# Nightmare-n/GD-MAE

Hardware: AMD Instinct MI355X
Metric: MAE pre-train frames/sec (Waymo-shape, 180k pts, 75% mask) (higher is better)
Workload: dtype bf16

## Files before the change

gd-mae_amd/csrc/vfe_fused.hip:

```cpp
#include "common.h"
#include "gemm.h"

int gd_bn_fold_from_partials(hipStream_t st, const float* part, int nblk, int C, double count, const float* gamma,
                             const float* beta, double eps, double momentum, float* running_mean, float* running_var,
                             long long* num_batches, double* stats, float* ab, float* mv);
int gd_partials_to_f64(hipStream_t st, const float* part, int nblk, int C2, double* out);
extern "C" int gdmae_bn_bwd_coeffs(const double* st, int n_st, const double* stats, const float* ab, const float* gamma, int C,
                                   double count, const double* tot, float* dgamma, float* dbeta, int accumulate, float* c01,
                                   void* stream);

namespace {

typedef float f32x16 __attribute__((ext_vector_type(16)));

constexpr int VF_C = 64;
constexpr int VF_WAVES = 4;
constexpr int VF_MAX_GRID = 1024;

struct VfeGeom {
  float lo[3], vs[3];
  int out_f16 = 0;
};

enum { VF_STATS = 0, VF_APPLY = 1, VF_BSTATS = 2, VF_DW = 3 };

__device__ inline unsigned short vf_f2bf(float f) { return gd_to_bf16(f); }

template <int F>
struct VfA {
  float r[F + 1];
  int pil;
};
struct VfB {
  long long c1, c2, c3;
  float m[3];
};
template <int F>
__device__ __forceinline__ void vf_load_a(const float* __restrict__ pts, const int* __restrict__ inv, long long i, long long N, VfA<F>& A) {
  const long long ic = i < N ? i : N - 1;
  const float* r = pts + ic * (F + 1);
#pragma unroll
  for (int k = 0; k < F + 1; ++k) A.r[k] = r[k];
  A.pil = inv[ic];
}
template <int F>
__device__ __forceinline__ void vf_load_b(const long long* __restrict__ coords, const float* __restrict__ mean, int cpp, long long i,
                                          long long N, int pil, VfB& B) {
  const long long ic = i < N ? i : N - 1;
  const long long* c = coords + 4 * (cpp ? (long long)pil : ic);
  const float* m = mean + (long long)pil * F;
  B.c1 = c[1]; B.c2 = c[2]; B.c3 = c[3];
  B.m[0] = m[0]; B.m[1] = m[1]; B.m[2] = m[2];
}
template <int F>
__device__ __forceinline__ void vf_features(const VfA<F>& A, const VfB& B, bool live, const VfeGeom& G, float (&f)[F + 6]) {
  const float x = A.r[1], y = A.r[2], z = A.r[3];
  f[0] = __fsub_rn(x, __fadd_rn(__fmul_rn(__fadd_rn((float)B.c3, 0.5f), G.vs[0]), G.lo[0]));
  f[1] = __fsub_rn(y, __fadd_rn(__fmul_rn(__fadd_rn((float)B.c2, 0.5f), G.vs[1]), G.lo[1]));
  f[2] = __fsub_rn(z, __fadd_rn(__fmul_rn(__fadd_rn((float)B.c1, 0.5f), G.vs[2]), G.lo[2]));
#pragma unroll
  for (int k = 0; k < F; ++k) f[3 + k] = A.r[1 + k];
  f[3 + F] = __fsub_rn(x, B.m[0]);
  f[4 + F] = __fsub_rn(y, B.m[1]);
  f[5 + F] = __fsub_rn(z, B.m[2]);
#pragma unroll
  for (int k = 0; k < F + 6; ++k) f[k] = live ? f[k] : 0.f;
}
template <bool BF>
struct VfG {
  unsigned u[BF ? 16 : 1];
  float2 v[BF ? 1 : 16];
};
template <bool BF>
__device__ __forceinline__ void vf_load_g(const void* __restrict__ g, long long base, long long N, int n, int half, VfG<BF>& Gr) {
#pragma unroll
  for (int r = 0; r < 16; ++r) {
    const long long row = base + 8 * (r / 4) + 4 * half + (r % 4);
    const long long rc = row < N ? row : N - 1;
    if (BF) Gr.u[r] = ((const unsigned*)g)[rc * (VF_C / 2) + n];
    else Gr.v[r] = ((const float2*)g)[rc * (VF_C / 2) + n];
  }
}

template <int F, int MODE, bool BF>
__global__ __launch_bounds__(VF_WAVES * 64) void k_vfe1(const float* __restrict__ pts, const long long* __restrict__ coords,
                                                        const int* __restrict__ inv, const float* __restrict__ mean,
                                                        int cpp, long long N, VfeGeom G, const float* __restrict__ W,
                                                        const float* __restrict__ ab, const float* __restrict__ c01,
                                                        const void* __restrict__ g, void* __restrict__ out,
                                                        float* __restrict__ part) {
  constexpr int D = F + 6;
  constexpr int KS = (D + 1) / 2;
  constexpr int DP = 2 * KS;
  const int lane = threadIdx.x & 63, wave = threadIdx.x >> 6;
  const int n = lane & 31, half = lane >> 5;
  __shared__ float sh[VF_WAVES * (MODE == VF_DW ? VF_C * D : 4 * VF_C)];
  __shared__ float shf[MODE == VF_DW ? VF_WAVES * 32 * DP : 1];

  float wb[2][KS];
#pragma unroll
  for (int blk = 0; blk < 2; ++blk)
#pragma unroll
    for (int s = 0; s < KS; ++s) {
      const int d = 2 * s + half;
      wb[blk][s] = d < D ? W[(2 * n + blk) * D + d] : 0.f;
    }
  float ca[2] = {0.f, 0.f}, cb[2] = {0.f, 0.f}, c0[2] = {0.f, 0.f}, c1[2] = {0.f, 0.f};
  if (MODE != VF_STATS) {
#pragma unroll
    for (int blk = 0; blk < 2; ++blk) {
      ca[blk] = ab[2 * n + blk];
      cb[blk] = ab[VF_C + 2 * n + blk];
      if (MODE == VF_DW) {
        c0[blk] = c01[2 * n + blk];
        c1[blk] = c01[VF_C + 2 * n + blk];
      }
    }
  }
  float s1[2] = {0.f, 0.f}, s2[2] = {0.f, 0.f};
  f32x16 accw[2];
#pragma unroll
  for (int r = 0; r < 16; ++r) accw[0][r] = accw[1][r] = 0.f;

  const long long ntiles = (N + 31) / 32;
  const long long tstride = (long long)gridDim.x * VF_WAVES;
  constexpr bool HAS_G = MODE == VF_BSTATS || MODE == VF_DW;
  constexpr bool PIPE = !HAS_G;
  VfA<F> A1, A2, A3;
  VfB B1, B2;
  VfG<BF> G1;
  if (PIPE) {
    const long long t = (long long)blockIdx.x * VF_WAVES + wave;
    vf_load_a<F>(pts, inv, t * 32 + n, N, A1);
    vf_load_a<F>(pts, inv, (t + tstride) * 32 + n, N, A2);
    vf_load_b<F>(coords, mean, cpp, t * 32 + n, N, A1.pil, B1);
  }
  for (long long t0 = (long long)blockIdx.x * VF_WAVES; t0 < ntiles; t0 += tstride) {
    const long long base = (t0 + wave) * 32;
    if (PIPE) {
      vf_load_a<F>(pts, inv, base + 2 * tstride * 32 + n, N, A3);
      vf_load_b<F>(coords, mean, cpp, base + tstride * 32 + n, N, A2.pil, B2);
      __builtin_amdgcn_sched_barrier(0);
    } else {
      vf_load_g<BF>(g, base, N, n, half, G1);
      vf_load_a<F>(pts, inv, base + n, N, A1);
      vf_load_b<F>(coords, mean, cpp, base + n, N, A1.pil, B1);
    }
    float g0[16], g1[16];
    if (HAS_G) {
#pragma unroll
      for (int r = 0; r < 16; ++r) {
        const long long row = base + 8 * (r / 4) + 4 * half + (r % 4);
        if (BF) {
          g0[r] = row < N ? __uint_as_float(G1.u[r] << 16) : 0.f;
          g1[r] = row < N ? __uint_as_float(G1.u[r] & 0xFFFF0000u) : 0.f;
        } else {
          g0[r] = row < N ? G1.v[r].x : 0.f;
          g1[r] = row < N ? G1.v[r].y : 0.f;
        }
      }
    }
    float f[D];
    vf_features<F>(A1, B1, base + n < N, G, f);
    f32x16 h[2];
#pragma unroll
    for (int r = 0; r < 16; ++r) h[0][r] = h[1][r] = 0.f;
#pragma unroll
    for (int s = 0; s < KS; ++s) {
      const float f0 = f[2 * s], f1 = (2 * s + 1 < D) ? f[2 * s + 1] : 0.f;
      const float a = half ? f1 : f0;
      h[0] = __builtin_amdgcn_mfma_f32_32x32x2f32(a, wb[0][s], h[0], 0, 0, 0);
      h[1] = __builtin_amdgcn_mfma_f32_32x32x2f32(a, wb[1][s], h[1], 0, 0, 0);
    }
    if (MODE == VF_STATS) {
#pragma unroll
      for (int r = 0; r < 16; ++r)
#pragma unroll
        for (int blk = 0; blk < 2; ++blk) {
          const float v = h[blk][r];
          s1[blk] += v;
          s2[blk] = fmaf(v, v, s2[blk]);
        }
    } else if (MODE == VF_APPLY) {
#pragma unroll
      for (int k = 0; k < F + 1; ++k) asm volatile("" : "+v"(A3.r[k]));
      asm volatile("" : "+v"(A3.pil));
      asm volatile("" : "+v"(B2.c1), "+v"(B2.c2), "+v"(B2.c3), "+v"(B2.m[0]), "+v"(B2.m[1]), "+v"(B2.m[2]));
#pragma unroll
      for (int r = 0; r < 16; ++r) {
        const long long row = base + 8 * (r / 4) + 4 * half + (r % 4);
        if (row < N) {
          const float y0 = fmaxf(fmaf(ca[0], h[0][r], cb[0]), 0.f), y1 = fmaxf(fmaf(ca[1], h[1][r], cb[1]), 0.f);
          if (BF) ((unsigned*)out)[row * (VF_C / 2) + n] = G.out_f16 ? gd_pack_f16(y0, y1) : ((unsigned)vf_f2bf(y0) | ((unsigned)vf_f2bf(y1) << 16));
          else ((float2*)out)[row * (VF_C / 2) + n] = make_float2(y0, y1);
        }
      }
    } else {
      if (MODE == VF_DW) {
        if (half == 0) {
#pragma unroll
          for (int d = 0; d < DP; ++d) shf[(wave * 32 + n) * DP + d] = d < D ? f[d] : 0.f;
        }
        __builtin_amdgcn_fence(__ATOMIC_RELEASE, "wavefront");
        __builtin_amdgcn_wave_barrier();
        __builtin_amdgcn_fence(__ATOMIC_ACQUIRE, "wavefront");
      }
#pragma unroll
      for (int r = 0; r < 16; ++r) {
        const int pr = 8 * (r / 4) + 4 * half + (r % 4);
        const float dh0 = fmaf(ca[0], h[0][r], cb[0]) > 0.f ? g0[r] : 0.f;
        const float dh1 = fmaf(ca[1], h[1][r], cb[1]) > 0.f ? g1[r] : 0.f;
        if (MODE == VF_BSTATS) {
          s1[0] += dh0;
          s1[1] += dh1;
          s2[0] = fmaf(dh0, h[0][r], s2[0]);
          s2[1] = fmaf(dh1, h[1][r], s2[1]);
        } else {
          const float dx0 = fmaf(c1[0], h[0][r], fmaf(ca[0], dh0, c0[0]));
          const float dx1 = fmaf(c1[1], h[1][r], fmaf(ca[1], dh1, c0[1]));
          const float bv = n < DP ? shf[(wave * 32 + pr) * DP + n] : 0.f;
          accw[0] = __builtin_amdgcn_mfma_f32_32x32x2f32(dx0, bv, accw[0], 0, 0, 0);
          accw[1] = __builtin_amdgcn_mfma_f32_32x32x2f32(dx1, bv, accw[1], 0, 0, 0);
        }
      }
      if (MODE == VF_DW) {
        __builtin_amdgcn_fence(__ATOMIC_RELEASE, "wavefront");
        __builtin_amdgcn_wave_barrier();
      }
    }
    if (PIPE) {
      A1 = A2;
      A2 = A3;
      B1 = B2;
    }
  }

  if (MODE == VF_STATS || MODE == VF_BSTATS) {
#pragma unroll
    for (int blk = 0; blk < 2; ++blk) {
      s1[blk] += __shfl_xor(s1[blk], 32, 64);
      s2[blk] += __shfl_xor(s2[blk], 32, 64);
    }
    if (half == 0) {
#pragma unroll
      for (int blk = 0; blk < 2; ++blk) {
        sh[wave * 2 * VF_C + 2 * n + blk] = s1[blk];
        sh[wave * 2 * VF_C + VF_C + 2 * n + blk] = s2[blk];
      }
    }
    __syncthreads();
    if (threadIdx.x < 2 * VF_C) {
      float a = 0.f;
#pragma unroll
      for (int w = 0; w < VF_WAVES; ++w) a += sh[w * 2 * VF_C + threadIdx.x];
      part[(long long)blockIdx.x * 2 * VF_C + threadIdx.x] = a;
    }
  } else if (MODE == VF_DW) {
    if (n < D) {
#pragma unroll
      for (int blk = 0; blk < 2; ++blk)
#pragma unroll
        for (int r = 0; r < 16; ++r) {
          const int col = 2 * (8 * (r / 4) + 4 * half + (r % 4)) + blk;
          sh[wave * VF_C * D + col * D + n] = accw[blk][r];
        }
    }
    __syncthreads();
    for (int e = threadIdx.x; e < VF_C * D; e += VF_WAVES * 64) {
      float a = 0.f;
#pragma unroll
      for (int w = 0; w < VF_WAVES; ++w) a += sh[w * VF_C * D + e];
      part[(long long)blockIdx.x * VF_C * D + e] = a;
    }
  }
}

template <typename K>
int vf_resident_blocks(K kernel, int slot) {
  static int cache[32] = {0};
  if (cache[slot] == 0) {
    int per_cu = 0, dev = 0;
    hipDeviceProp_t prop;
    if (hipOccupancyMaxActiveBlocksPerMultiprocessor(&per_cu, kernel, VF_WAVES * 64, 0) != hipSuccess || per_cu < 1) per_cu = 2;
    if (hipGetDevice(&dev) != hipSuccess || hipGetDeviceProperties(&prop, dev) != hipSuccess) prop.multiProcessorCount = 256;
    const long long b = (long long)per_cu * prop.multiProcessorCount;
    cache[slot] = (int)(b > VF_MAX_GRID ? VF_MAX_GRID : b);
  }
  return cache[slot];
}

template <int MODE>
int vf_launch(hipStream_t st, int F, bool bf, const float* pts, const long long* coords, const int* inv, const float* mean,
              int cpp, long long N, const VfeGeom& G, const float* W, const float* ab, const float* c01, const void* g, void* out,
              float* part, int* grid_out = nullptr) {
  const long long tiles = (N + 31) / 32, blocks = (tiles + VF_WAVES - 1) / VF_WAVES;
  const dim3 block(VF_WAVES * 64);
#define VF_GO(FF, BB)                                                                                                   \
  do {                                                                                                                  \
    const int cap = vf_resident_blocks(k_vfe1<FF, MODE, BB>, ((FF - 3) * 4 + MODE) * 2 + (BB ? 1 : 0));                 \
    const dim3 grid((unsigned)(blocks < cap ? blocks : cap));                                                           \
    if (grid_out) *grid_out = (int)grid.x;                                                                              \
    hipLaunchKernelGGL((k_vfe1<FF, MODE, BB>), grid, block, 0, st, pts, coords, inv, mean, cpp, N, G, W, ab, c01, g, out, part); \
  } while (0)
  if (F == 5) { if (bf) VF_GO(5, true); else VF_GO(5, false); }
  else if (F == 4) { if (bf) VF_GO(4, true); else VF_GO(4, false); }
  else if (F == 3) { if (bf) VF_GO(3, true); else VF_GO(3, false); }
  else GD_REQUIRE(false, "vfe point layer: 3, 4 or 5 point features (x, y, z [, intensity [, elongation]])");
#undef VF_GO
  GD_LAUNCH_CHECK();
  return 0;
}

}

__global__ __launch_bounds__(256) void k_pillar_major_rows(const float* __restrict__ pts, int ncols, const int* __restrict__ csr,
                                                           const int* __restrict__ inv, const int* __restrict__ n_dev,
                                                           float* __restrict__ pts_pm, int* __restrict__ rowpil) {
  const long long N = *n_dev;
  for (long long q = blockIdx.x * (long long)blockDim.x + threadIdx.x; q < N; q += (long long)gridDim.x * blockDim.x) {
    const int i = csr[q];
    rowpil[q] = inv[i];
    for (int k = 0; k < ncols; ++k) pts_pm[q * ncols + k] = pts[(long long)i * ncols + k];
  }
}

extern "C" int gdmae_pillar_major_rows(const float* points, int n_cols, const int* pillar_pts, const int* inverse32,
                                       const int* n_dev, long long capacity, float* points_pm, int* row_pillar,
                                       void* stream) {
  if (capacity <= 0) return 0;
  hipLaunchKernelGGL(k_pillar_major_rows, dim3((unsigned)(capacity / 256 + 1 > 8192 ? 8192 : capacity / 256 + 1)), dim3(256), 0, (hipStream_t)stream, points, n_cols,
                     pillar_pts, inverse32, n_dev, points_pm, row_pillar);
  GD_LAUNCH_CHECK();
  return 0;
}

extern "C" size_t gdmae_vfe_point_layer_workspace_bytes(int n_cols) {
  const int D = n_cols - 1 + 6;
  return gd_align((size_t)VF_MAX_GRID * VF_C * (D > 2 ? D : 2) * sizeof(float)) + gd_align(2 * VF_C * sizeof(double)) +
         gd_align(2 * VF_C * sizeof(float));
}

extern "C" int gdmae_vfe_point_layer_fwd(const float* points, const long long* point_coords, const int* inverse32,
                                         const float* pillar_mean, int coords_per_pillar, long long N, int n_cols,
                                         const float* lo, const float* vs,
                                         const float* W, int C, const float* gamma, const float* beta, double eps,
                                         double momentum, float* running_mean, float* running_var, long long* num_batches,
                                         double* stats, float* ab, float* mv, void* out, int out_bf16, void* workspace,
                                         void* stream) {
  GD_REQUIRE(C == VF_C, "vfe point layer: 64 output channels");
  GD_REQUIRE(N > 0, "vfe point layer: no points");
  hipStream_t st = (hipStream_t)stream;
  VfeGeom G;
  for (int i = 0; i < 3; ++i) { G.lo[i] = lo[i]; G.vs[i] = vs[i]; }
  float* part = (float*)workspace;
  const int F = n_cols - 1;
  int grid = 0;
  int rc = vf_launch<VF_STATS>(st, F, false, points, point_coords, inverse32, pillar_mean, coords_per_pillar, N, G, W, nullptr, nullptr, nullptr,
                               nullptr, part, &grid);
  if (rc) return rc;
  rc = gd_bn_fold_from_partials(st, part, grid, C, (double)N, gamma, beta, eps, momentum, running_mean, running_var,
                                num_batches, stats, ab, mv);
  if (rc) return rc;
  G.out_f16 = out_bf16 == 2;
  return vf_launch<VF_APPLY>(st, F, out_bf16 != 0, points, point_coords, inverse32, pillar_mean, coords_per_pillar, N, G, W, ab, nullptr, nullptr,
                             out, nullptr);
}

extern "C" int gdmae_vfe_point_layer_bwd(const float* points, const long long* point_coords, const int* inverse32,
                                         const float* pillar_mean, int coords_per_pillar, long long N, int n_cols,
                                         const float* lo, const float* vs,
                                         const float* W, int C, const float* gamma, const double* stats, const float* ab,
                                         const void* g, int g_bf16, float* dgamma, float* dbeta, float* dW, int accumulate,
                                         void* workspace, void* stream) {
  GD_REQUIRE(C == VF_C, "vfe point layer: 64 output channels");
  GD_REQUIRE(N > 0, "vfe point layer: no points");
  hipStream_t st = (hipStream_t)stream;
  VfeGeom G;
  for (int i = 0; i < 3; ++i) { G.lo[i] = lo[i]; G.vs[i] = vs[i]; }
  const int F = n_cols - 1, D = F + 6;
  char* p = (char*)workspace;
  float* part = (float*)p;
  p += gd_align((size_t)VF_MAX_GRID * VF_C * (D > 2 ? D : 2) * sizeof(float));
  double* sums = (double*)p;
  p += gd_align(2 * VF_C * sizeof(double));
  float* c01 = (float*)p;
  int grid = 0;
  int rc = vf_launch<VF_BSTATS>(st, F, g_bf16 != 0, points, point_coords, inverse32, pillar_mean, coords_per_pillar, N, G, W, ab, nullptr, g,
                                nullptr, part, &grid);
  if (rc) return rc;
  rc = gd_partials_to_f64(st, part, grid, 2 * C, sums);
  if (rc) return rc;
  rc = gdmae_bn_bwd_coeffs(sums, 2, stats, ab, gamma, C, (double)N, nullptr, dgamma, dbeta, accumulate, c01, stream);
  if (rc) return rc;
  rc = vf_launch<VF_DW>(st, F, g_bf16 != 0, points, point_coords, inverse32, pillar_mean, coords_per_pillar, N, G, W, ab, c01, g, nullptr, part, &grid);
  if (rc) return rc;
  return gd_splitk_acc(st, part, grid, (long long)VF_C * D, dW, accumulate);
}
```

Baseline: 1056.

## Fuse VFE point-layer backward into single pass using feature Gram matrix

```diff
diff --git a/gd-mae_amd/csrc/vfe_fused.hip b/gd-mae_amd/csrc/vfe_fused.hip
--- a/gd-mae_amd/csrc/vfe_fused.hip
+++ b/gd-mae_amd/csrc/vfe_fused.hip
@@ -1,28 +1,26 @@
 #include "common.h"
-#include "gemm.h"
 
 int gd_bn_fold_from_partials(hipStream_t st, const float* part, int nblk, int C, double count, const float* gamma,
                              const float* beta, double eps, double momentum, float* running_mean, float* running_var,
                              long long* num_batches, double* stats, float* ab, float* mv);
-int gd_partials_to_f64(hipStream_t st, const float* part, int nblk, int C2, double* out);
-extern "C" int gdmae_bn_bwd_coeffs(const double* st, int n_st, const double* stats, const float* ab, const float* gamma, int C,
-                                   double count, const double* tot, float* dgamma, float* dbeta, int accumulate, float* c01,
-                                   void* stream);
 
 namespace {
 
 typedef float f32x16 __attribute__((ext_vector_type(16)));
+typedef float f32x4 __attribute__((ext_vector_type(4)));
 
 constexpr int VF_C = 64;
 constexpr int VF_WAVES = 4;
 constexpr int VF_MAX_GRID = 1024;
+constexpr int VF_FS = 16;
+constexpr int vf_bwd_part(int D) { return (VF_C + D + 1) * (D + 1); }
 
 struct VfeGeom {
   float lo[3], vs[3];
   int out_f16 = 0;
 };
 
-enum { VF_STATS = 0, VF_APPLY = 1, VF_BSTATS = 2, VF_DW = 3 };
+enum { VF_STATS = 0, VF_APPLY = 1, VF_BWD = 2 };
 
 __device__ inline unsigned short vf_f2bf(float f) { return gd_to_bf16(f); }
 
@@ -86,16 +84,16 @@
 __global__ __launch_bounds__(VF_WAVES * 64) void k_vfe1(const float* __restrict__ pts, const long long* __restrict__ coords,
                                                         const int* __restrict__ inv, const float* __restrict__ mean,
                                                         int cpp, long long N, VfeGeom G, const float* __restrict__ W,
-                                                        const float* __restrict__ ab, const float* __restrict__ c01,
-                                                        const void* __restrict__ g, void* __restrict__ out,
+                                                        const float* __restrict__ ab, const void* __restrict__ g, void* __restrict__ out,
                                                         float* __restrict__ part) {
   constexpr int D = F + 6;
   constexpr int KS = (D + 1) / 2;
-  constexpr int DP = 2 * KS;
   const int lane = threadIdx.x & 63, wave = threadIdx.x >> 6;
   const int n = lane & 31, half = lane >> 5;
-  __shared__ float sh[VF_WAVES * (MODE == VF_DW ? VF_C * D : 4 * VF_C)];
-  __shared__ float shf[MODE == VF_DW ? VF_WAVES * 32 * DP : 1];
+  constexpr int DQ = D + 1, PW = vf_bwd_part(D);
+  static_assert(DQ <= VF_FS, "feature tile row");
+  __shared__ float sh[VF_WAVES * (MODE == VF_BWD ? PW : 4 * VF_C)];
+  __shared__ __attribute__((aligned(16))) float shf[MODE == VF_BWD ? VF_WAVES * 32 * VF_FS : 4];
 
   float wb[2][KS];
 #pragma unroll
@@ -105,26 +103,26 @@
       const int d = 2 * s + half;
       wb[blk][s] = d < D ? W[(2 * n + blk) * D + d] : 0.f;
     }
-  float ca[2] = {0.f, 0.f}, cb[2] = {0.f, 0.f}, c0[2] = {0.f, 0.f}, c1[2] = {0.f, 0.f};
+  float ca[2] = {0.f, 0.f}, cb[2] = {0.f, 0.f};
   if (MODE != VF_STATS) {
 #pragma unroll
     for (int blk = 0; blk < 2; ++blk) {
       ca[blk] = ab[2 * n + blk];
       cb[blk] = ab[VF_C + 2 * n + blk];
-      if (MODE == VF_DW) {
-        c0[blk] = c01[2 * n + blk];
-        c1[blk] = c01[VF_C + 2 * n + blk];
-      }
     }
   }
   float s1[2] = {0.f, 0.f}, s2[2] = {0.f, 0.f};
   f32x16 accw[2];
 #pragma unroll
   for (int r = 0; r < 16; ++r) accw[0][r] = accw[1][r] = 0.f;
+  f32x4 accf = {0.f, 0.f, 0.f, 0.f};
+  float sft[F];
+#pragma unroll
+  for (int k = 0; k < F; ++k) sft[k] = MODE == VF_BWD ? pts[1 + k] : 0.f;
 
   const long long ntiles = (N + 31) / 32;
   const long long tstride = (long long)gridDim.x * VF_WAVES;
-  constexpr bool HAS_G = MODE == VF_BSTATS || MODE == VF_DW;
+  constexpr bool HAS_G = MODE == VF_BWD;
   constexpr bool PIPE = !HAS_G;
   VfA<F> A1, A2, A3;
   VfB B1, B2;
@@ -147,16 +145,18 @@
       vf_load_b<F>(coords, mean, cpp, base + n, N, A1.pil, B1);
     }
     float g0[16], g1[16];
+    const long long left = N - base;
+    const int nrem = left < 0 ? 0 : (left > 32 ? 32 : (int)left);
     if (HAS_G) {
 #pragma unroll
       for (int r = 0; r < 16; ++r) {
-        const long long row = base + 8 * (r / 4) + 4 * half + (r % 4);
+        const bool ok = 8 * (r / 4) + 4 * half + (r % 4) < nrem;
         if (BF) {
-          g0[r] = row < N ? __uint_as_float(G1.u[r] << 16) : 0.f;
-          g1[r] = row < N ? __uint_as_float(G1.u[r] & 0xFFFF0000u) : 0.f;
+          g0[r] = ok ? __uint_as_float(G1.u[r] << 16) : 0.f;
+          g1[r] = ok ? __uint_as_float(G1.u[r] & 0xFFFF0000u) : 0.f;
         } else {
-          g0[r] = row < N ? G1.v[r].x : 0.f;
-          g1[r] = row < N ? G1.v[r].y : 0.f;
+          g0[r] = ok ? G1.v[r].x : 0.f;
+          g1[r] = ok ? G1.v[r].y : 0.f;
         }
       }
     }
@@ -196,37 +196,37 @@
         }
       }
     } else {
-      if (MODE == VF_DW) {
-        if (half == 0) {
-#pragma unroll
-          for (int d = 0; d < DP; ++d) shf[(wave * 32 + n) * DP + d] = d < D ? f[d] : 0.f;
-        }
-        __builtin_amdgcn_fence(__ATOMIC_RELEASE, "wavefront");
-        __builtin_amdgcn_wave_barrier();
-        __builtin_amdgcn_fence(__ATOMIC_ACQUIRE, "wavefront");
-      }
+      if (half == 0) {
+        const bool live = n < nrem;
+        float t[VF_FS];
+#pragma unroll
+        for (int d = 0; d < VF_FS; ++d) t[d] = d < D ? f[d] : (d == D && live ? 1.f : 0.f);
+#pragma unroll
+        for (int k = 0; k < F; ++k) t[3 + k] = live ? __fsub_rn(f[3 + k], sft[k]) : 0.f;
+#pragma unroll
+        for (int q = 0; q < VF_FS / 4; ++q)
+          ((float4*)shf)[(wave * 32 + n) * (VF_FS / 4) + q] = make_float4(t[4 * q], t[4 * q + 1], t[4 * q + 2], t[4 * q + 3]);
+      }
+      __builtin_amdgcn_fence(__ATOMIC_RELEASE, "wavefront");
+      __builtin_amdgcn_wave_barrier();
+      __builtin_amdgcn_fence(__ATOMIC_ACQUIRE, "wavefront");
+      int tb = (wave * 32 + 4 * half) * VF_FS + (n & (VF_FS - 1));
+      asm volatile("" : "+v"(tb));
 #pragma unroll
       for (int r = 0; r < 16; ++r) {
-        const int pr = 8 * (r / 4) + 4 * half + (r % 4);
         const float dh0 = fmaf(ca[0], h[0][r], cb[0]) > 0.f ? g0[r] : 0.f;
         const float dh1 = fmaf(ca[1], h[1][r], cb[1]) > 0.f ? g1[r] : 0.f;
-        if (MODE == VF_BSTATS) {
-          s1[0] += dh0;
-          s1[1] += dh1;
-          s2[0] = fmaf(dh0, h[0][r], s2[0]);
-          s2[1] = fmaf(dh1, h[1][r], s2[1]);
-        } else {
-          const float dx0 = fmaf(c1[0], h[0][r], fmaf(ca[0], dh0, c0[0]));
-          const float dx1 = fmaf(c1[1], h[1][r], fmaf(ca[1], dh1, c0[1]));
-          const float bv = n < DP ? shf[(wave * 32 + pr) * DP + n] : 0.f;
-          accw[0] = __builtin_amdgcn_mfma_f32_32x32x2f32(dx0, bv, accw[0], 0, 0, 0);
-          accw[1] = __builtin_amdgcn_mfma_f32_32x32x2f32(dx1, bv, accw[1], 0, 0, 0);
-        }
-      }
-      if (MODE == VF_DW) {
-        __builtin_amdgcn_fence(__ATOMIC_RELEASE, "wavefront");
-        __builtin_amdgcn_wave_barrier();
-      }
+        const float bv = shf[tb + (8 * (r / 4) + (r % 4)) * VF_FS];
+        accw[0] = __builtin_amdgcn_mfma_f32_32x32x2f32(dh0, bv, accw[0], 0, 0, 0);
+        accw[1] = __builtin_amdgcn_mfma_f32_32x32x2f32(dh1, bv, accw[1], 0, 0, 0);
+      }
+#pragma unroll
+      for (int s = 0; s < 8; ++s) {
+        const float tv = shf[wave * 32 * VF_FS + s * 64 + lane];
+        accf = __builtin_amdgcn_mfma_f32_16x16x4f32(tv, tv, accf, 0, 0, 0);
+      }
+      __builtin_amdgcn_fence(__ATOMIC_RELEASE, "wavefront");
+      __builtin_amdgcn_wave_barrier();
     }
     if (PIPE) {
       A1 = A2;
@@ -235,7 +235,7 @@
     }
   }
 
-  if (MODE == VF_STATS || MODE == VF_BSTATS) {
+  if (MODE == VF_STATS) {
 #pragma unroll
     for (int blk = 0; blk < 2; ++blk) {
       s1[blk] += __shfl_xor(s1[blk], 32, 64);
@@ -255,29 +255,34 @@
       for (int w = 0; w < VF_WAVES; ++w) a += sh[w * 2 * VF_C + threadIdx.x];
       part[(long long)blockIdx.x * 2 * VF_C + threadIdx.x] = a;
     }
-  } else if (MODE == VF_DW) {
-    if (n < D) {
+  } else if (MODE == VF_BWD) {
+    if (n < DQ) {
 #pragma unroll
       for (int blk = 0; blk < 2; ++blk)
 #pragma unroll
         for (int r = 0; r < 16; ++r) {
           const int col = 2 * (8 * (r / 4) + 4 * half + (r % 4)) + blk;
-          sh[wave * VF_C * D + col * D + n] = accw[blk][r];
+          sh[wave * PW + col * DQ + n] = accw[blk][r];
         }
     }
+#pragma unroll
+    for (int r = 0; r < 4; ++r) {
+      const int i = 4 * (lane >> 4) + r, j = lane & 15;
+      if (i < DQ && j < DQ) sh[wave * PW + (VF_C + i) * DQ + j] = accf[r];
+    }
     __syncthreads();
-    for (int e = threadIdx.x; e < VF_C * D; e += VF_WAVES * 64) {
+    for (int e = threadIdx.x; e < PW; e += VF_WAVES * 64) {
       float a = 0.f;
 #pragma unroll
-      for (int w = 0; w < VF_WAVES; ++w) a += sh[w * VF_C * D + e];
-      part[(long long)blockIdx.x * VF_C * D + e] = a;
+      for (int w = 0; w < VF_WAVES; ++w) a += sh[w * PW + e];
+      part[(long long)blockIdx.x * PW + e] = a;
     }
   }
 }
 
 template <typename K>
 int vf_resident_blocks(K kernel, int slot) {
-  static int cache[32] = {0};
+  static int cache[18] = {0};
   if (cache[slot] == 0) {
     int per_cu = 0, dev = 0;
     hipDeviceProp_t prop;
@@ -291,16 +296,16 @@
 
 template <int MODE>
 int vf_launch(hipStream_t st, int F, bool bf, const float* pts, const long long* coords, const int* inv, const float* mean,
-              int cpp, long long N, const VfeGeom& G, const float* W, const float* ab, const float* c01, const void* g, void* out,
+              int cpp, long long N, const VfeGeom& G, const float* W, const float* ab, const void* g, void* out,
               float* part, int* grid_out = nullptr) {
   const long long tiles = (N + 31) / 32, blocks = (tiles + VF_WAVES - 1) / VF_WAVES;
   const dim3 block(VF_WAVES * 64);
 #define VF_GO(FF, BB)                                                                                                   \
   do {                                                                                                                  \
-    const int cap = vf_resident_blocks(k_vfe1<FF, MODE, BB>, ((FF - 3) * 4 + MODE) * 2 + (BB ? 1 : 0));                 \
+    const int cap = vf_resident_blocks(k_vfe1<FF, MODE, BB>, ((FF - 3) * 3 + MODE) * 2 + (BB ? 1 : 0));                 \
     const dim3 grid((unsigned)(blocks < cap ? blocks : cap));                                                           \
     if (grid_out) *grid_out = (int)grid.x;                                                                              \
-    hipLaunchKernelGGL((k_vfe1<FF, MODE, BB>), grid, block, 0, st, pts, coords, inv, mean, cpp, N, G, W, ab, c01, g, out, part); \
+    hipLaunchKernelGGL((k_vfe1<FF, MODE, BB>), grid, block, 0, st, pts, coords, inv, mean, cpp, N, G, W, ab, g, out, part); \
   } while (0)
   if (F == 5) { if (bf) VF_GO(5, true); else VF_GO(5, false); }
   else if (F == 4) { if (bf) VF_GO(4, true); else VF_GO(4, false); }
@@ -311,6 +316,67 @@
   return 0;
 }
 
+constexpr int VF_FIN_CH = 8, VF_FIN_SL = 4, VF_FIN_E = 256;
+__global__ __launch_bounds__(VF_FIN_SL * VF_FIN_E) void k_vfe1_finish(const float* __restrict__ part, int S, int D,
+                                                                      const float* __restrict__ pts, const float* __restrict__ W,
+                                                                      const double* __restrict__ stats, const float* __restrict__ ab,
+                                                                      const float* __restrict__ gamma, double count,
+                                                                      float* __restrict__ dgamma, float* __restrict__ dbeta,
+                                                                      float* __restrict__ dW, int accumulate) {
+  __shared__ double sh[VF_FIN_SL][VF_FIN_E];
+  __shared__ double T[VF_FIN_E];
+  const int DQ = D + 1, PW = (VF_C + DQ) * DQ, E = VF_FIN_CH * DQ + DQ * DQ;
+  const int e = threadIdx.x % VF_FIN_E, sl = threadIdx.x / VF_FIN_E;
+  {
+    const int ec = e < E ? e : E - 1;
+    const float* p = part + (ec < VF_FIN_CH * DQ ? blockIdx.x * VF_FIN_CH * DQ + ec : VF_C * DQ + (ec - VF_FIN_CH * DQ));
+    const int s0 = (S * sl) / VF_FIN_SL, s1 = (S * (sl + 1)) / VF_FIN_SL;
+    double acc = 0.0;
+    for (int b0 = s0; b0 < s1; b0 += 16) {
+      float v[16];
+#pragma unroll
+      for (int u = 0; u < 16; ++u) v[u] = p[(long long)(b0 + u < s1 ? b0 + u : s1 - 1) * PW];
+#pragma unroll
+      for (int u = 0; u < 16; ++u) acc += b0 + u < s1 ? (double)v[u] : 0.0;
+    }
+    sh[sl][e] = acc;
+  }
+  __syncthreads();
+  if (threadIdx.x < VF_FIN_E) {
+    double a = 0.0;
+#pragma unroll
+    for (int k = 0; k < VF_FIN_SL; ++k) a += sh[k][threadIdx.x];
+    T[threadIdx.x] = a;
+  }
+  __syncthreads();
+  if (threadIdx.x >= VF_FIN_CH * D) return;
+  const int cl = threadIdx.x / D, d = threadIdx.x % D, c = blockIdx.x * VF_FIN_CH + cl;
+  const double* Pc = T + cl * DQ;
+  const double* M = T + VF_FIN_CH * DQ;
+  auto shift = [&](int k) { return k >= 3 && k < D - 3 ? (double)pts[k - 2] : 0.0; };
+  const double db = Pc[D];
+  double dhh = 0.0, wff = 0.0;
+  const double sd = shift(d), fsd = M[D * DQ + d] + count * sd;
+  for (int k = 0; k < D; ++k) {
+    const double w = (double)W[c * D + k], sk = shift(k);
+    dhh += w * (Pc[k] + db * sk);
+    wff += w * (M[k * DQ + d] + sk * M[D * DQ + d] + M[D * DQ + k] * sd + count * sk * sd);
+  }
+  const double mean = stats[c], r = stats[VF_C + c], a = (double)ab[c];
+  const double da = dhh - db * mean;
+  const double dv = -0.5 * (da * (double)gamma[c]) * r * r * r;
+  const double dmu = -db * a - 2.0 * mean * dv;
+  const double c0 = dmu / count, c1 = 2.0 * dv / count;
+  const float dw = (float)(a * (Pc[d] + db * sd) + c0 * fsd + c1 * wff);
+  if (accumulate) dW[c * D + d] += dw;
+  else dW[c * D + d] = dw;
+  if (d == 0) {
+    const float dg = (float)(da * r), dbf = (float)db;
+    if (accumulate) { dgamma[c] += dg; dbeta[c] += dbf; }
+    else { dgamma[c] = dg; dbeta[c] = dbf; }
+  }
+}
+
 }
 
 __global__ __launch_bounds__(256) void k_pillar_major_rows(const float* __restrict__ pts, int ncols, const int* __restrict__ csr,
@@ -335,9 +401,8 @@
 }
 
 extern "C" size_t gdmae_vfe_point_layer_workspace_bytes(int n_cols) {
-  const int D = n_cols - 1 + 6;
-  return gd_align((size_t)VF_MAX_GRID * VF_C * (D > 2 ? D : 2) * sizeof(float)) + gd_align(2 * VF_C * sizeof(double)) +
-         gd_align(2 * VF_C * sizeof(float));
+  const int D = n_cols - 1 + 6, pw = vf_bwd_part(D > 0 ? D : 0);
+  return gd_align((size_t)VF_MAX_GRID * (pw > 2 * VF_C ? pw : 2 * VF_C) * sizeof(float));
 }
 
 extern "C" int gdmae_vfe_point_layer_fwd(const float* points, const long long* point_coords, const int* inverse32,
@@ -355,14 +420,14 @@
   float* part = (float*)workspace;
   const int F = n_cols - 1;
   int grid = 0;
-  int rc = vf_launch<VF_STATS>(st, F, false, points, point_coords, inverse32, pillar_mean, coords_per_pillar, N, G, W, nullptr, nullptr, nullptr,
+  int rc = vf_launch<VF_STATS>(st, F, false, points, point_coords, inverse32, pillar_mean, coords_per_pillar, N, G, W, nullptr, nullptr,
                                nullptr, part, &grid);
   if (rc) return rc;
   rc = gd_bn_fold_from_partials(st, part, grid, C, (double)N, gamma, beta, eps, momentum, running_mean, running_var,
                                 num_batches, stats, ab, mv);
   if (rc) return rc;
   G.out_f16 = out_bf16 == 2;
-  return vf_launch<VF_APPLY>(st, F, out_bf16 != 0, points, point_coords, inverse32, pillar_mean, coords_per_pillar, N, G, W, ab, nullptr, nullptr,
+  return vf_launch<VF_APPLY>(st, F, out_bf16 != 0, points, point_coords, inverse32, pillar_mean, coords_per_pillar, N, G, W, ab, nullptr,
                              out, nullptr);
 }
 
@@ -378,21 +443,13 @@
   VfeGeom G;
   for (int i = 0; i < 3; ++i) { G.lo[i] = lo[i]; G.vs[i] = vs[i]; }
   const int F = n_cols - 1, D = F + 6;
-  char* p = (char*)workspace;
-  float* part = (float*)p;
-  p += gd_align((size_t)VF_MAX_GRID * VF_C * (D > 2 ? D : 2) * sizeof(float));
-  double* sums = (double*)p;
-  p += gd_align(2 * VF_C * sizeof(double));
-  float* c01 = (float*)p;
+  float* part = (float*)workspace;
   int grid = 0;
-  int rc = vf_launch<VF_BSTATS>(st, F, g_bf16 != 0, points, point_coords, inverse32, pillar_mean, coords_per_pillar, N, G, W, ab, nullptr, g,
-                                nullptr, part, &grid);
+  int rc = vf_launch<VF_BWD>(st, F, g_bf16 != 0, points, point_coords, inverse32, pillar_mean, coords_per_pillar, N, G, W, ab, g, nullptr,
+                             part, &grid);
   if (rc) return rc;
-  rc = gd_partials_to_f64(st, part, grid, 2 * C, sums);
-  if (rc) return rc;
-  rc = gdmae_bn_bwd_coeffs(sums, 2, stats, ab, gamma, C, (double)N, nullptr, dgamma, dbeta, accumulate, c01, stream);
-  if (rc) return rc;
-  rc = vf_launch<VF_DW>(st, F, g_bf16 != 0, points, point_coords, inverse32, pillar_mean, coords_per_pillar, N, G, W, ab, c01, g, nullptr, part, &grid);
-  if (rc) return rc;
-  return gd_splitk_acc(st, part, grid, (long long)VF_C * D, dW, accumulate);
-}
+  hipLaunchKernelGGL(k_vfe1_finish, dim3(VF_C / VF_FIN_CH), dim3(VF_FIN_SL * VF_FIN_E), 0, st, part, grid, D, points, W, stats, ab, gamma,
+                     (double)N, dgamma, dbeta, dW, accumulate);
+  GD_LAUNCH_CHECK();
+  return 0;
+}
```

Result: no change. 1064, median of 6 (+0.7%).
